# simeonjunker/retr

Measured on AMD Instinct MI355X. Metric: RefCOCO images/sec (train fwd+bwd) at 1/2/4/8 GPUs; greedy-decode refs/sec, higher is better.
Workload: dtype bf16; 1 GPU; cfg2: ResNet-50 + 6-enc/6-dec d_model 256, 640x640, batch 16/GPU, fwd+CE+bwd+allreduce+clip+AdamW; global_batch=16, seq_len=128, parallelism=dp1

## Files before the change

include/retr_hip.h:

```cpp
#ifndef RETR_HIP_H
#define RETR_HIP_H
#include <stddef.h>
#ifdef __cplusplus
extern "C" {
#endif

#define RETR_DTYPE_F32 0
#define RETR_DTYPE_BF16 1

const char* retr_last_error(void);
int retr_abi_version(void);
void retr_set_seed_base(const unsigned long long* device_ptr);
void retr_set_deterministic(int on);
int retr_get_deterministic(void);
int retr_seed_bump(unsigned long long* device_ptr, unsigned long long delta, void* stream);
int retr_spin_us(float us, void* stream);

int retr_linear_fwd(int dtype, const void* x, long ldx, const void* w, long ldw,
                    const float* bias, void* y, long ldy, int y_f32, int M, int N, int K, int relu,
                    const float* residual, long ldr, float drop_p, unsigned long long seed,
                    void* stream);
int retr_linear_dgrad(int dtype, const void* dy, long lddy, const void* w, long ldw, void* dx,
                      long lddx, int dx_f32, int M, int N, int K, const void* addend,
                      int addend_f32, long lda, const void* gate, long ldg, int w_trans,
                      void* stream);
int retr_linear_splits(int dtype, int M, int N, int K);
int retr_linear_fwd_splitk(int dtype, const void* x, long ldx, const void* w, long ldw,
                           const float* bias, void* y, long ldy, int y_f32, int M, int N, int K,
                           int relu, const float* residual, long ldr, float drop_p,
                           unsigned long long seed, float* ws, int splits, void* stream);

typedef struct retr_ln_out {
  const float* gamma;
  const float* beta;
  float eps;
  int y_bf16;
  void* y;
  void* y2;
  long ldy;
  const float* pos;
  int period;
  float* mean;
  float* rstd;
} retr_ln_out;
int retr_linear_fwd_splitk_ln(int dtype, const void* x, long ldx, const void* w, long ldw,
                              const float* bias, float* y, long ldy, int M, int N, int K, int relu,
                              const float* residual, long ldr, float drop_p,
                              unsigned long long seed, float* ws, int splits,
                              const retr_ln_out* ln, void* stream);
int retr_linear_dgrad_splitk(int dtype, const void* dy, long lddy, const void* w, long ldw,
                             void* dx, long lddx, int dx_f32, int M, int N, int K,
                             const void* addend, int addend_f32, long lda, const void* gate,
                             long ldg, int w_trans, float* ws, int splits, void* stream);
int retr_linear_dgrad_slabs(int dtype, const void* dy, long lddy, const void* w, long ldw, int M,
                            int N, int K, int w_trans, float* ws, int splits, void* stream);
int retr_linear_wgrad(int dtype, const void* dy, long lddy, const void* x, long ldx, float* dw,
                      long lddw, int M, int N, int K, float* db, int accumulate, void* stream);
int retr_bias_grad(int dtype, const void* dy, long lddy, int M, int N, float* db, void* stream);

enum {
  RETR_TUNE_GROUP_TILE = 0,
  RETR_TUNE_GROUP_STAGES = 1,
  RETR_TUNE_WGRAD_TILE = 2,
  RETR_TUNE_WGRAD_STAGES = 3,
  RETR_TUNE_WGRAD_KC = 4,
  RETR_TUNE_ATTN_MODE = 5,
  RETR_TUNE_BIG_TILE = 6,
  RETR_TUNE_NT_STORE = 7,
  RETR_TUNE_CONV_WGRAD_SPLITS = 8,
  RETR_TUNE_CONV_WGRAD_TILE = 9,
  RETR_TUNE_ATTN_SPLIT = 10,
  RETR_TUNE_LIN_WGRAD = 11,
  RETR_TUNE_ATTN_FSPLIT = 12,
  RETR_TUNE_LIN_SMALL = 13,
  RETR_TUNE_SHORTK = 14,
  RETR_TUNE_ADAMW_NT = 15,
  RETR_TUNE_WGRAD_B32 = 16,
  RETR_TUNE_WGRAD_FUSED = 17,
  RETR_TUNE_SPLITK_FUSED = 18,
  RETR_TUNE_WB_CHUNK = 19,
  RETR_TUNE_CW_CHUNK = 20,
  RETR_TUNE_CONV3X3 = 21,
  RETR_TUNE_C3_TILE = 22,
  RETR_TUNE_PANEL = 23,
  RETR_TUNE_PANEL_GROUPS = 24,
  RETR_TUNE_PANEL_CONV = 25,
  RETR_TUNE_ATTN_KEEPPRE = 26,
  RETR_TUNE_LN_BWD = 27,
  RETR_TUNE_UNPACK_GRID = 28,
  RETR_TUNE_CW_WAVES = 29,
  RETR_TUNE_DEC_ORDER = 30,
  RETR_TUNE_DEC_WAVES = 31,
  RETR_TUNE_ROWLN = 32,
  RETR_TUNE_LIN_K256 = 33,
  RETR_TUNE_COUNT = 40
};
int retr_tune(int knob, int value);

typedef struct {
  const void* x; long ldx;
  const void* w; long ldw;
  const float* bias;
  void* y; long ldy;
  const float* residual; long ldr;
  float drop_p; unsigned long long seed;
  int M, N, K, relu;
} retr_linear_fwd_desc;
int retr_linear_fwd_group(int dtype, int y_f32, int n, const retr_linear_fwd_desc* d,
                          void* stream);

typedef struct {
  const void* dy; long lddy;
  const void* w; long ldw;
  void* dx; long lddx;
  const void* addend; long lda;
  const void* gate; long ldg;
  int M, N, K, pad;
} retr_linear_dgrad_desc;
int retr_linear_dgrad_group(int dtype, int dx_f32, int addend_f32, int w_trans, int n,
                            const retr_linear_dgrad_desc* d, void* stream);

typedef struct {
  const void* dy; long lddy;
  const void* x; long ldx;
  float* dw; long lddw;
  float* db;
  int M, N, K, accumulate;
} retr_linear_wgrad_desc;
size_t retr_linear_wgrad_group_workspace(int n, const retr_linear_wgrad_desc* d);
int retr_linear_wgrad_group(int dtype, int n, const retr_linear_wgrad_desc* d, void* workspace,
                            void* stream);
typedef struct {
  const float* parts;
  long stride;
  int nparts, cols;
  float* dst;
  int accumulate;
} retr_slab_sum_desc;
int retr_linear_wgrad_group2(int dtype, int n, const retr_linear_wgrad_desc* d, void* workspace,
                             int nx, const retr_slab_sum_desc* x, void* stream);
size_t retr_linear_wgrad_batch_table_bytes(int n, int nx);
int retr_linear_wgrad_batch(int n, const retr_linear_wgrad_desc* d, int nx,
                            const retr_slab_sum_desc* x, void* table, size_t table_bytes,
                            void* stream);

int retr_ffn_splits(int M, int C, int F);
int retr_ffn_fwd(const void* n, long ldn, const void* w1, const float* b1, const void* w2,
                 const float* b2, void* h, long ldh, const float* residual, long ldr, float* y,
                 long ldy, int M, int C, int F, float drop_p, unsigned long long seed, float* ws,
                 int splits, void* stream);
int retr_ffn_bwd_data(const void* dbr, long lddbr, const void* w2, const void* h, long ldh,
                      const void* w1, void* dh, long lddh, void* dn, long lddn, int M, int C,
                      int F, float* ws, int splits, void* stream);

int retr_conv_pack(int dtype, const float* w, const float* bn_w, const float* bn_b,
                   const float* bn_rm, const float* bn_rv, const float* conv_bias, int Co, int Ci,
                   int KH, int KW, int Cp, void* w_out, void* wt_out, float* bias_out,
                   float* scale_out, void* stream);
typedef struct {
  const float *w, *bn_w, *bn_b, *bn_rm, *bn_rv, *conv_bias;
  void *w_out, *wt_out;
  float *bias_out, *scale_out;
  int Co, Ci, KH, KW, Cp, pad;
} retr_conv_pack_desc;
int retr_conv_pack_group(int dtype, int n, const retr_conv_pack_desc* d, void* stream);
typedef struct {
  const void *a, *b;
  void* dst;
  const float *bias_a, *bias_b;
  float* bias_dst;
  int rows, ka, kb;
} retr_cat_rows_desc;
int retr_cat_rows_group(int n, const retr_cat_rows_desc* d, void* stream);
int retr_conv2d_fwd(int dtype, const void* x, int Nb, int H, int W, int C, const void* w,
                    const float* bias, const void* residual, void* y, int Co, int KH, int KW,
                    int stride, int pad, int dil, int relu, void* stream);
int retr_conv2d_fwd_out(int dtype, const void* x, int Nb, int H, int W, int C, const void* w,
                        const float* bias, const void* residual, void* y, int Co, int KH, int KW,
                        int stride, int pad, int dil, int OH, int OW, int relu, void* stream);
int retr_conv1x1_fwd_cat(int dtype, const void* x1, int C1, const void* x2, int C2, int Nb,
                         int OH, int OW, int H2, int W2, int stride2, const void* w,
                         const float* bias, void* y, int Co, int relu, void* stream);
int retr_conv2d_dgrad(int dtype, const void* dy, int Nb, int H, int W, int C, const void* wt,
                      void* dx, int Co, int KH, int KW, int stride, int pad, int dil,
                      const void* addend, const void* gate, void* stream);
int retr_conv2d_wgrad(int dtype, const void* dy, const void* x, int Nb, int H, int W, int C,
                      float* ws, int Co, int KH, int KW, int stride, int pad, int dil,
                      void* stream);
int retr_conv2d_wgrad_splits(int dtype, int Nb, int H, int W, int C, int Co, int KH, int KW,
                             int stride, int pad, int dil);
typedef struct {
  const void* dy; const void* x;
  float* ws;
  int Nb, H, W, C, Co, KH, KW, stride, pad, dil;
  int splits, kind;
} retr_conv_wgrad_desc;
size_t retr_conv2d_wgrad_group_table_bytes(int n);
int retr_conv2d_wgrad_group_plan(int dtype, int n, retr_conv_wgrad_desc* d);
int retr_conv2d_wgrad_group(int dtype, int n, const retr_conv_wgrad_desc* d, void* table,
                            size_t table_bytes, void* stream);
typedef struct {
  const float* ws; const float* scale;
  float* grad;
  int Co, Ci, Cp, KH, KW, splits, accumulate, pad;
} retr_conv_unpack_desc;
size_t retr_conv_wgrad_unpack_group_table_bytes(int n);
int retr_conv_wgrad_unpack_group(int n, const retr_conv_unpack_desc* d, void* table,
                                 size_t table_bytes, void* stream);
int retr_conv_wgrad_unpack(const float* ws, const float* scale, float* grad, int Co, int Ci,
                           int Cp, int KH, int KW, int accumulate, int splits, void* stream);
int retr_bottleneck_s1_fwd(int dtype, const void* x, int N, int H, int W, int Cin,
                           const void* w1, const float* b1, const void* w2, const float* b2,
                           const void* w3, const float* b3, int ds, void* y, void* stream);
int retr_stem_pool_fwd(int dtype, const void* x, int N, int H2, int W2, const void* w,
                       const float* bias, void* y, int Co, void* stream);
int retr_nchw_to_nhwc(int dtype, const float* x, void* y, int N, int C, int H, int W, int Cp,
                      void* stream);
int retr_nchw_to_s2d16(const float* x, void* y, int N, int C, int H, int W, void* stream);
int retr_stem_s2d_weights(const void* wp, void* w2, int Co, int Cp, void* stream);
typedef struct {
  long long src_off;
  long long tmp_off;
  int H, W;
  int x0, y0, rw, rh;
  int bx, by, bw, bh;
  int D, ox, oy;
  int mx, my;
  int coef_off, ksize;
  int win_off;
  int ops;
  float f[3];
  int pad_[2];
} retr_pipe_item;
int retr_pipe_run(const unsigned char* src, const retr_pipe_item* items, int n, const int* coef,
                  const int* win, unsigned char* tmp, int max_d, unsigned char* u8, float* out,
                  unsigned char* mask, int S, const float* mean, const float* std_,
                  void* stream);
int retr_maxpool3x3s2(int dtype, const void* x, void* y, int N, int H, int W, int C, int OH,
                      int OW, void* stream);
int retr_mask_nearest(const unsigned char* m, unsigned char* out, int N, int H, int W, int h,
                      int w, void* stream);

int retr_layernorm_fwd(int dtype, const float* x, long ldx, const float* gamma,
                       const float* beta, float eps, int M, int C, void* y, long ldy, void* y2,
                       const float* pos, int period, float* mean, float* rstd, void* stream);
int retr_layernorm_bwd(int dtype, const void* dy, const void* dy2, long lddy, const float* x,
                       long ldx, const float* gamma, const float* mean, const float* rstd, int M,
                       int C, float* dx, long lddx, const float* addend, float* dgamma,
                       float* dbeta, float* workspace, void* stream);
size_t retr_layernorm_bwd_workspace(int M, int C);
int retr_layernorm_bwd2(int dtype, const void* dy, const void* dy2, long lddy, const float* x,
                        long ldx, const float* gamma, const float* mean, const float* rstd, int M,
                        int C, float* dx, long lddx, const float* addend, float* dgamma,
                        float* dbeta, float* workspace, void* dxd, long lddxd, float drop_p,
                        unsigned long long seed, int* nparts, void* stream);
int retr_layernorm_bwd_slabs(const float* ws, int splits, const float* x, long ldx,
                             const float* gamma, const float* mean, const float* rstd, int M,
                             int C, float* dx, long lddx, const float* addend, float* dgamma,
                             float* dbeta, float* workspace, void* dxd, long lddxd, float drop_p,
                             unsigned long long seed, int* nparts, void* stream);

int retr_embed_ln_fwd(const long long* tokens, int B, int T, int C, const float* word,
                      const float* posw, const float* gamma, const float* beta, float eps,
                      float drop_p, unsigned long long seed, float* y, float* mean, float* rstd,
                      void* stream);
int retr_embed_ln_bwd(const long long* tokens, int B, int T, int C, const float* word,
                      const float* posw, const float* gamma, const float* mean, const float* rstd,
                      const float* dy, float drop_p, unsigned long long seed, float* dword,
                      float* dposw, float* dgamma, float* dbeta, int padding_idx,
                      void* workspace, void* stream);
size_t retr_embed_ln_bwd_workspace(int B, int T, int C);

int retr_attention_fwd(int dtype, const void* q, long ldq, const void* k, long ldk,
                       const void* v, long ldv, void* o, long ldo, int B, int H, int Lq, int Lk,
                       int hd, const unsigned char* kpm, int causal, float drop_p,
                       unsigned long long seed, float* lse, float* probs, void* stream);
int retr_attention_bwd(int dtype, const void* q, long ldq, const void* k, long ldk,
                       const void* v, long ldv, const void* o, long ldo, const void* dout,
                       long lddo, const float* lse, void* dq, long lddq, void* dk, long lddk,
                       void* dv, long lddv, int B, int H, int Lq, int Lk, int hd,
                       const unsigned char* kpm, int causal, float drop_p,
                       unsigned long long seed, float* workspace, void* stream);
size_t retr_attention_bwd_workspace(int B, int H, int Lq);
size_t retr_attention_dropout_mask_bytes(int B, int H, int Lq, int Lk);
int retr_attention_fwd_dm(int dtype, const void* q, long ldq, const void* k, long ldk,
                          const void* v, long ldv, void* o, long ldo, int B, int H, int Lq,
                          int Lk, int hd, const unsigned char* kpm, int causal, float drop_p,
                          unsigned long long seed, float* lse, float* probs, void* dmask,
                          void* stream);
int retr_attention_bwd_dm(int dtype, const void* q, long ldq, const void* k, long ldk,
                          const void* v, long ldv, const void* o, long ldo, const void* dout,
                          long lddo, const float* lse, void* dq, long lddq, void* dk, long lddk,
                          void* dv, long lddv, int B, int H, int Lq, int Lk, int hd,
                          const unsigned char* kpm, int causal, float drop_p,
                          unsigned long long seed, float* workspace, const void* dmask,
                          void* stream);
int retr_attention_decode(int dtype, const void* q, long ldq, const void* k, long ldk,
                          const void* v, long ldv, void* o, long ldo, int B, int H, int Lk,
                          int Lmax, int hd, const unsigned char* kpm, int kv_group,
                          const int* anc, void* stream);

int retr_ce_fwd(int dtype, const void* logits, long ld, int M, int V, const long long* targets,
                float* lse, float* loss_rows, float* loss, void* stream);
int retr_ce_bwd(int dtype, const void* logits, long ld, int M, int V, const long long* targets,
                const float* lse, const float* dloss, float inv_count, void* dlogits, long lddl,
                void* stream);
int retr_ce_fwd_bwd(int dtype, const void* logits, long ld, int M, int V,
                    const long long* targets, float* lse, float* loss_rows, float* loss,
                    float inv_count, void* dlogits, long lddl, void* stream);
int retr_ce_bwd_rescale(int dtype, const void* logits, long ld, int M, int V,
                        const long long* targets, const float* lse, const float* dloss,
                        float inv_count, void* dlogits, long lddl, void* stream);
int retr_ce_count(int M, const long long* targets, long long ignore_index, float* denom,
                  void* stream);
int retr_ce_fwd_opt(int dtype, const void* logits, long ld, int M, int V,
                    const long long* targets, long long ignore_index, float label_smoothing,
                    float* lse, float* loss_rows, float* loss, const float* denom,
                    void* stream);
int retr_ce_bwd_opt(int dtype, const void* logits, long ld, int M, int V,
                    const long long* targets, long long ignore_index, float label_smoothing,
                    const float* lse, const float* dloss, long dloss_stride, const float* denom,
                    void* dlogits, long lddl, void* stream);
int retr_ce_fwd_bwd_opt(int dtype, const void* logits, long ld, int M, int V,
                        const long long* targets, long long ignore_index, float label_smoothing,
                        float* lse, float* loss_rows, float* loss, const float* denom,
                        void* dlogits, long lddl, void* stream);
int retr_ce_bwd_rescale_opt(int dtype, const void* logits, long ld, int M, int V,
                            const long long* targets, long long ignore_index,
                            float label_smoothing, const float* lse, const float* dloss,
                            const float* denom, void* dlogits, long lddl, void* stream);
int retr_argmax_rows(int dtype, const void* x, long ld, int M, int V, long long* out,
                     void* stream);
size_t retr_argmax_workspace(int M);
int retr_argmax_rows_ws(int dtype, const void* x, long ld, int M, int V, long long* out,
                        void* workspace, void* stream);

int retr_topk_rows(int dtype, const void* x, long ld, int M, int V, int K, int* idx,
                   float* logprob, void* stream);
int retr_beam_select(const int* cand_tok, const float* cand_lp, int B, int K, int i, int T,
                     long long eos, float* scores, unsigned char* finished, long long* hist,
                     int* anc, long long* tok, unsigned char* item_done, int* done,
                     void* stream);
int retr_greedy_update(const long long* pred, int B, int T, int i, long long eos,
                       long long* caption, unsigned char* finished, int* done, long long* tok,
                       void* stream);
int retr_greedy_select(int dtype, const void* logits, long ld, int B, int V, void* workspace,
                       int T, int i, long long eos, long long* pred, long long* caption,
                       unsigned char* finished, int* done, long long* tok, void* stream);
int retr_greedy_select2(int dtype, const void* logits, long ld, int B, int V, void* workspace,
                        int T, int i, long long eos, long long* pred, long long* caption,
                        unsigned char* finished, int* done, long long* tok, int write_all,
                        void* stream);

int retr_add_pos_fwd(int dtype, const float* x, long ldx, int M, int C, const float* pos,
                     int period, void* y, void* y2, long ldy, void* stream);
int retr_sum2(int dtype, const void* a, const void* b, long n, float* out, void* stream);
int retr_dropout_apply(int dtype_out, const float* x, long ldx, void* y, long ldy, int M, int N,
                       float drop_p, unsigned long long seed, void* stream);
int retr_transpose_cast(int dtype, const float* x, void* y, int R, int C, int R_pad,
                        void* stream);
int retr_cast(int dtype, const float* x, void* y, long n, void* stream);
int retr_pos_grad(int dtype, const void* d, long ld, int M, int C, int period, float* dpos,
                  void* stream);
int retr_pos_grad_set(int dtype, const void* d, long ld, int M, int C, int period, float* dpos,
                      void* stream);
typedef struct retr_pos_item {
  const void* d;
  long ld;
  int M;
  int pad;
} retr_pos_item;
int retr_pos_grad_multi(int dtype, int n, const retr_pos_item* items, int C, int period,
                        float* dpos, int accumulate, void* stream);

int retr_adamw_sumsq(const float* grad, long n, float* partials, int nparts, float* step,
                     void* stream);
int retr_adamw_update(float* param, float* grad, float* exp_avg, float* exp_avg_sq, long n,
                      const float* hyper, double beta1, double beta2, float eps,
                      const float* step, float step_offset, const float* partials, int nparts,
                      float max_norm, void* param_bf16, void* stream);
int retr_adamw_update2(float* param, float* grad, float* exp_avg, float* exp_avg_sq, long n,
                       const float* hyper, double beta1, double beta2, float eps,
                       const float* step, float step_offset, const float* partials, int nparts,
                       float max_norm, void* param_bf16, int zero_grad, void* stream);

int retr_dec_gemm(const void* a_plain, const void* a_pos, int R, int C, const void* w,
                  const float* bias, int N, void* d0, long rs0, int pos0, void* d1, long rs1,
                  int pos1, void* d2, long rs2, int pos2, int segw, int relu, void* stream);
int retr_dec_rows(const float* xin, const float* slabs, int nslab, const float* b2, int R, int C,
                  float* xout, const float* gamma, const float* beta, float eps, const float* pos,
                  void* n, void* npos, void* stream);
int retr_dec_embed_rows(const long long* tok, int R, int C, const float* word, const float* qpos,
                        const float* ge, const float* be, float epse, float* x, const float* g1,
                        const float* b1, float eps1, void* n, void* npos, void* stream);
int retr_dec_attn_row(const void* q, const void* k, const void* v, int R, int C, int H, int Lk,
                      int Lmax, int kv_group, const int* anc, const unsigned char* kpm,
                      const float* x, const void* wo, const float* bo, float* xo,
// ... 82 lines not shown
```

retr_amd/csrc/conv.hip:

```cpp
#include <algorithm>
#include <cstring>
#include <vector>

#include "gemm2.hpp"
#include "panel.hpp"
#include "epilogues.hpp"
#include "../../include/retr_hip.h"

using namespace retr;

namespace retr {
bool conv3x3_direct_ok(int H, int W, int CI, int CO);
int conv3x3_fwd_direct(const bf16* x, const bf16* w, const float* bias, bf16* y, int relu, int Nb,
                       int H, int W, int CI, int CO, hipStream_t st);
int conv3x3_dgrad_direct(const bf16* dy, const bf16* wt, bf16* dx, const bf16* addend,
                         const bf16* gate, int Nb, int H, int W, int CI_out, int CO_in,
                         hipStream_t st);
}

namespace {

struct Geom {
  int Nb, H, W, C, Co, KH, KW, s, p, d, OH, OW;
};
// ... 245 lines not shown
    int hw = g.OH * g.OW;
    const int n = m / hw;
    int rem = m - n * hw;
    k.oh = rem / g.OW;
    k.ow = rem - k.oh * g.OW;
    k.base = (((long)n * g.H + k.oh * g.s) * g.W + k.ow * g.s) * g.C;
    return k;
  }
  RETR_DEVICE void advance(KCur& k, int d) const {
    k.m += d;
    if (d != Elem<T>::BK) {
      k = kcur(k.m);
      return;
    }
    const long rowC = (long)g.s * g.W * g.C;
    k.ow += adv_r;
    k.oh += adv_q;
    k.base += (long)adv_q * rowC + (long)adv_r * g.s * g.C;
    if (k.ow >= g.OW) {
      k.ow -= g.OW;
      k.oh += 1;
      k.base += rowC - (long)g.OW * g.s * g.C;
    }
    while (k.oh >= g.OH) {
      k.oh -= g.OH;
      k.base += ((long)g.H - (long)g.OH * g.s) * g.W * g.C;
    }
  }
  RETR_DEVICE const void* addr(const Ctx& c, const KCur& k) const {
    if (!c.ok || k.m >= M) return nullptr;
    int ih = k.oh * g.s + c.khd, iw = k.ow * g.s + c.kwd;
    if ((unsigned)ih >= (unsigned)g.H || (unsigned)iw >= (unsigned)g.W) return nullptr;
    return x + k.base + c.off;
  }
};

template <typename T>
struct ConvWgradB32 {
  static constexpr bool kContig = false;
  const T* x;
  Geom g;
  int rows, M;
  int adv_q, adv_r;
  int d_step, d_row, d_img;
  struct Ctx { int khd, kwd, off; bool ok; };
  struct KCur { int m, oh, ow, base; };
  RETR_DEVICE Ctx row_ctx(int r) const {
    Ctx c;
    c.ok = r < rows;
    const int rr = c.ok ? r : 0;
    const int khw = rr / g.C;
    const int ci = rr - khw * g.C;
    const int kh = khw / g.KW, kw = khw - kh * g.KW;
    c.khd = kh * g.d - g.p;
    c.kwd = kw * g.d - g.p;
    c.off = (c.khd * g.W + c.kwd) * g.C + ci;
    return c;
  }
  RETR_DEVICE KCur kcur(int m) const {
    KCur k;
    k.m = m;
    const int hw = g.OH * g.OW;
    const int n = m / hw;
    const int rem = m - n * hw;
    k.oh = rem / g.OW;
    k.ow = rem - k.oh * g.OW;
    k.base = ((n * g.H + k.oh * g.s) * g.W + k.ow * g.s) * g.C;
    return k;
  }
  RETR_DEVICE void advance(KCur& k, int d) const {
    if (d != Elem<T>::BK) {
      k = kcur(k.m + d);
      return;
    }
    k.m += d;
    k.ow += adv_r;
    k.oh += adv_q;
    k.base += d_step;
    if (k.ow >= g.OW) {
      k.ow -= g.OW;
      k.oh += 1;
      k.base += d_row;
    }
    if (k.oh >= g.OH) {
      k.oh -= g.OH;
      k.base += d_img;
    }
  }
  RETR_DEVICE bool ok(const Ctx& c, const KCur& k) const {
    const int ih = k.oh * g.s + c.khd, iw = k.ow * g.s + c.kwd;
    return c.ok & (k.m < M) & ((unsigned)ih < (unsigned)g.H) & ((unsigned)iw < (unsigned)g.W);
  }
  RETR_DEVICE const void* addr(const Ctx& c, const KCur& k) const {
    return ok(c, k) ? (const void*)(x + (unsigned)(k.base + c.off)) : nullptr;
  }
  RETR_DEVICE const void* addr_or(const Ctx& c, const KCur& k, const void* fb) const {
    return ok(c, k) ? (const void*)(x + (unsigned)(k.base + c.off)) : fb;
  }
};

struct Phase {
  int a, b;
  int ih0, iw0;
  int Hp, Wp;
  int nkh, nkw;
};

template <typename T>
struct ConvDgradPhaseA {
  static constexpr bool kContig = true;
  const T* gr;
  Geom g;
  Phase ph;
  int M, K;
  struct Ctx { const T* img; int i, j; bool ok; };
  struct KCur { int k, c, ti, tj; };
  RETR_DEVICE Ctx row_ctx(int r) const {
    Ctx c;
    c.ok = r < M;
    const int rr = c.ok ? r : 0;
    const int hw = ph.Hp * ph.Wp;
    const int n = rr / hw, rem = rr - n * hw;
    c.i = rem / ph.Wp;
    c.j = rem - c.i * ph.Wp;
    c.img = gr + (long)n * g.OH * g.OW * g.Co;
    return c;
  }
  RETR_DEVICE KCur kcur(int k) const {
    KCur t;
    t.k = k;
    const int tap = k / g.Co;
    t.c = k - tap * g.Co;
    t.ti = tap / ph.nkw;
    t.tj = tap - t.ti * ph.nkw;
    return t;
  }
  RETR_DEVICE void advance(KCur& t, int d) const {
    t.k += d;
    t.c += d;
    while (t.c >= g.Co) {
      t.c -= g.Co;
      if (++t.tj == ph.nkw) {
        t.tj = 0;
        ++t.ti;
      }
    }
  }
  RETR_DEVICE const void* addr(const Ctx& c, const KCur& t) const {
    if (!c.ok || t.k >= K) return nullptr;
    const int oh = c.i + ((ph.ih0 + g.p - ph.a) >> 1) - t.ti;
    const int ow = c.j + ((ph.iw0 + g.p - ph.b) >> 1) - t.tj;
    if ((unsigned)oh >= (unsigned)g.OH || (unsigned)ow >= (unsigned)g.OW) return nullptr;
    return c.img + ((long)oh * g.OW + ow) * g.Co + t.c;
  }
};

template <typename T>
struct ConvDgradPhaseAU {
  static constexpr bool kContig = true;
  static constexpr bool kUniformK = true;
  const T* gr;
  Geom g;
  Phase ph;
  int M, K;
  struct Ctx { const T* base; unsigned mask; };
  struct KCur { int c0, t, ti, tj, off; };
  RETR_DEVICE Ctx row_ctx_c(int r, int coff) const {
    Ctx c;
    const bool ok = r < M;
    const int rr = ok ? r : 0;
    const int hw = ph.Hp * ph.Wp;
    const int n = rr / hw, rem = rr - n * hw;
    const int i = rem / ph.Wp, j = rem - i * ph.Wp;
    const int oh0 = i + ((ph.ih0 + g.p - ph.a) >> 1), ow0 = j + ((ph.iw0 + g.p - ph.b) >> 1);
    c.base = gr + (((long)n * g.OH + oh0) * g.OW + ow0) * g.Co + coff;
    unsigned m = 0;
    if (ok) {
      for (int ti = 0; ti < ph.nkh; ++ti)
        for (int tj = 0; tj < ph.nkw; ++tj)
          if ((unsigned)(oh0 - ti) < (unsigned)g.OH && (unsigned)(ow0 - tj) < (unsigned)g.OW)
            m |= 1u << (ti * ph.nkw + tj);
    }
    c.mask = m;
    return c;
  }
  RETR_DEVICE Ctx row_ctx(int r) const { return row_ctx_c(r, 0); }
  RETR_DEVICE void set_off(KCur& t) const { t.off = t.c0 - (t.ti * g.OW + t.tj) * g.Co; }
  RETR_DEVICE KCur kcur(int k) const {
    KCur t;
    t.t = k / g.Co;
    t.c0 = k - t.t * g.Co;
    t.ti = t.t / ph.nkw;
    t.tj = t.t - t.ti * ph.nkw;
    set_off(t);
    return t;
  }
  RETR_DEVICE void advance(KCur& t, int d) const {
    t.c0 += d;
    if (t.c0 >= g.Co) {
      t.c0 -= g.Co;
      ++t.t;
      if (++t.tj == ph.nkw) {
        t.tj = 0;
        ++t.ti;
      }
    }
    set_off(t);
  }
  RETR_DEVICE const void* addr(const Ctx& c, const KCur& t) const {
    if (!((c.mask >> t.t) & 1u)) return nullptr;
    return c.base + t.off;
  }
  RETR_DEVICE const void* addr_or(const Ctx& c, const KCur& t, const void* fb) const {
    return ((c.mask >> t.t) & 1u) ? (const void*)(c.base + t.off) : fb;
  }
};

template <typename T>
struct DgradPhaseWU {
  static constexpr bool kContig = true;
  static constexpr bool kUniformK = true;
  const T* wt;
  Geom g;
  Phase ph;
  int rows, K;
  struct Ctx { const T* row; int klim; };
  struct KCur { int k, c0, ti, tj, off; };
  RETR_DEVICE Ctx row_ctx_c(int r, int coff) const {
    return Ctx{wt + (long)(r < rows ? r : 0) * g.KH * g.KW * g.Co + coff, r < rows ? K : 0};
  }
  RETR_DEVICE Ctx row_ctx(int r) const { return row_ctx_c(r, 0); }
  RETR_DEVICE void set_off(KCur& t) const {
    t.off = ((ph.a + 2 * t.ti) * g.KW + ph.b + 2 * t.tj) * g.Co + t.c0;
  }
  RETR_DEVICE KCur kcur(int k) const {
    KCur t;
    t.k = k;
    const int tap = k / g.Co;
    t.c0 = k - tap * g.Co;
    t.ti = tap / ph.nkw;
    t.tj = tap - t.ti * ph.nkw;
    set_off(t);
    return t;
  }
  RETR_DEVICE void advance(KCur& t, int d) const {
    t.k += d;
    t.c0 += d;
    if (t.c0 >= g.Co) {
      t.c0 -= g.Co;
      if (++t.tj == ph.nkw) {
        t.tj = 0;
        ++t.ti;
      }
    }
    set_off(t);
  }
  RETR_DEVICE const void* addr(const Ctx& c, const KCur& t) const {
    return t.k < c.klim ? (const void*)(c.row + t.off) : nullptr;
  }
  RETR_DEVICE const void* addr_or(const Ctx& c, const KCur& t, const void* fb) const {
    return t.k < c.klim ? (const void*)(c.row + t.off) : fb;
  }
};

template <typename T>
struct DgradPhaseW {
  static constexpr bool kContig = true;
  const T* wt;
  Geom g;
  Phase ph;
  int rows, K;
  struct Ctx { const T* row; bool ok; };
  struct KCur { int k, c, ti, tj; };
  RETR_DEVICE Ctx row_ctx(int r) const {
    return Ctx{wt + (long)(r < rows ? r : 0) * g.KH * g.KW * g.Co, r < rows};
  }
  RETR_DEVICE KCur kcur(int k) const {
    KCur t;
    t.k = k;
    const int tap = k / g.Co;
    t.c = k - tap * g.Co;
    t.ti = tap / ph.nkw;
    t.tj = tap - t.ti * ph.nkw;
    return t;
  }
  RETR_DEVICE void advance(KCur& t, int d) const {
    t.k += d;
    t.c += d;
    while (t.c >= g.Co) {
      t.c -= g.Co;
      if (++t.tj == ph.nkw) {
        t.tj = 0;
        ++t.ti;
      }
    }
  }
  RETR_DEVICE const void* addr(const Ctx& c, const KCur& t) const {
    if (!c.ok || t.k >= K) return nullptr;
    const int kh = ph.a + 2 * t.ti, kw = ph.b + 2 * t.tj;
    return c.row + ((long)kh * g.KW + kw) * g.Co + t.c;
  }
};

template <class EP>
struct EpiPhaseRows {
  EP ep;
  int Hp, Wp, H, W, ih0, iw0;
  static constexpr bool kRowSum = false;
  float* rowsum = nullptr;
  RETR_DEVICE int map(int m) const {
    const int hw = Hp * Wp;
    const int n = m / hw, rem = m - n * hw;
    const int i = rem / Wp, j = rem - i * Wp;
    return (n * H + ih0 + 2 * i) * W + iw0 + 2 * j;
  }
  RETR_DEVICE void apply(int m, int n, float v) const { ep.apply(map(m), n, v); }
  RETR_DEVICE void apply8(int m, int n, float (&v)[8]) const { ep.apply8(map(m), n, v); }
  using Pre = typename EP::Pre;
  RETR_DEVICE void fetch8(int m, int n, Pre& p) const { ep.fetch8(map(m), n, p); }
  RETR_DEVICE void apply8p(int m, int n, float (&v)[8], const Pre& p) const {
    ep.apply8p(map(m), n, v, p);
  }
  RETR_DEVICE void empty_split(int, int) const {}
  RETR_DEVICE bool lane_contiguous() const { return false; }
};

inline bool prefer_tile64(int M, int N, int K, bool dense1x1, bool res_small_k) {
  if (retr_tune_get(RETR_TUNE_BIG_TILE) != 0) return false;
  if (res_small_k) return true;
  if (M <= 8192 && (N <= 512 || K <= 512)) return true;
  return dense1x1 && N >= 1024 && K <= 512 && M <= 32768;
}

template <int FAM, typename T, class LA, class LB, class EP>
int launch_auto(const LA& la, const LB& lb, const EP& ep, int M, int N, int K, int splits,
                hipStream_t st, const char* what, bool dense1x1 = false,
                bool res_small_k = false) {
  if constexpr (sizeof(T) == 2) {
    return launch_big<FAM>(la, lb, ep, M, N, K, splits, st, what,
                           prefer_tile64(M, N, K, dense1x1, res_small_k));
  } else {
    if (N >= 128 && M >= 4096) return launch_gemm<FAM, T, 128, 128>(la, lb, ep, M, N, K, splits, st, what);
    return launch_gemm<FAM, T, 64, 64>(la, lb, ep, M, N, K, splits, st, what);
  }
}

struct WgradPlan {
  int tile;
  int splits;
};

template <typename T>
WgradPlan wgrad_plan(int R, int Ncols, int Mp, bool dense1x1) {
  constexpr int BK = Elem<T>::BK;
  WgradPlan p{64, 1};
  if (R >= 128 && Ncols >= 128) p.tile = sizeof(T) == 2 ? 128 : 129;
  const int tt = retr_tune_get(RETR_TUNE_CONV_WGRAD_TILE);
  if (sizeof(T) == 2 && R >= 64 && Ncols >= 64 &&
      (tt == 1 || (tt == 0 && dense1x1 && (R <= 128 || Ncols <= 128 || Mp <= 8192))))
    p.tile = 65;
  if (p.tile == 65 && tt == 3) p.tile = 66;
  const int bm = (p.tile == 64 || p.tile == 65 || p.tile == 66) ? 64 : 128;
  const int bn = bm;
  const long tiles = (long)cdiv(R, bm) * cdiv(Ncols, bn);
  const int ksteps = cdiv(Mp, BK);
  const int tune = retr_tune_get(RETR_TUNE_CONV_WGRAD_SPLITS);
  long smax = ksteps / 8;
  if (smax > 128) smax = 128;
  if (smax < 1) smax = 1;
  long s;
  if (tune >= 2) {
    s = tune < smax ? tune : smax;
  } else if (tune == 1 || (p.tile != 128 && p.tile != 65 && p.tile != 66)) {
    s = (512 + tiles - 1) / tiles;
    if (s > smax) s = smax;
  } else {
    const long slots = p.tile == 66 ? 2048 : p.tile == 65 ? 1024 : 512;
    const double slab_cost = p.tile == 128 ? 0.016 : 0.004;
    s = 1;
    double best = 1e30;
    for (long c = 1; c <= smax; ++c) {
      const long kc = cdiv(ksteps, (int)c);
      const long rounds = (tiles * cdiv(ksteps, (int)kc) + slots - 1) / slots;
      const double cost = (double)rounds * (kc + 2) + slab_cost * (double)tiles * c;
      if (cost < best) { best = cost; s = c; }
    }
  }
  if (s < 1) s = 1;
  const int kchunk = cdiv(ksteps, (int)s) * BK;
  p.splits = cdiv(Mp, kchunk);
  return p;
}

template <int FAM, typename T, class LA, class LB>
int launch_wgrad(const LA& la, const LB& lb, float* ws, long ldws, int R, int Ncols, int Mp,
                 hipStream_t st, const char* what, bool dense1x1) {
  const WgradPlan p = wgrad_plan<T>(R, Ncols, Mp, dense1x1);
  const int s = p.splits;
  EpiAccF32 ep{ws, ldws, 0, 0, 1, nullptr};
  ep.split_stride = s > 1 ? (long)R * ldws : 0;
  ep.set_vec();
  if constexpr (sizeof(T) == 2) {
    if (p.tile == 128 && !dense1x1)
      return launch_gemm2<FAM, 128, 128, 4, 2, 2>(la, lb, ep, R, Ncols, Mp, s, st, what);
    if (p.tile == 128) return launch_gemm2<FAM, 128, 128, 2, 2, 2>(la, lb, ep, R, Ncols, Mp, s, st, what);
    if (p.tile == 65) return launch_gemm2<FAM, 64, 64, 2, 2, 2>(la, lb, ep, R, Ncols, Mp, s, st, what);
    if (p.tile == 66) return launch_gemm2<FAM, 64, 64, 2, 2, 1>(la, lb, ep, R, Ncols, Mp, s, st, what);
  } else {
    if (p.tile == 129) return launch_gemm<FAM, T, 128, 128>(la, lb, ep, R, Ncols, Mp, s, st, what);
  }
  return launch_gemm<FAM, T, 64, 64>(la, lb, ep, R, Ncols, Mp, s, st, what);
}

template <typename T>
int conv_fwd_t(const void* x, Geom g, const void* w, const float* bias, const void* res, void* y,
               int relu, hipStream_t st) {
  int M = g.Nb * g.OH * g.OW, N = g.Co, K = g.KH * g.KW * g.C;
  DenseK<T> lb{(const T*)w, (long)K, N, K};
  EpiFwd<T, T> ep{(T*)y, (long)N, bias, (const T*)res, (long)N, relu ? 2 : 0, DropoutParams{0, 0, 1.f}, 0};
  ep.set_vec();
  if (g.KH == 1 && g.KW == 1 && g.s == 1 && g.p == 0) {
    DenseK<T> la{(const T*)x, (long)g.C, M, K};
    if constexpr (sizeof(T) == 2) {
      if (K <= 256 && K % 64 == 0 && N >= 1024 && retr_tune_get(RETR_TUNE_PANEL) == 1 &&
          retr_tune_get(RETR_TUNE_PANEL_CONV) == 1)
        return launch_panel<kFamConvFwd>(la, lb, ep, M, N, K, st, "conv_fwd_1x1");
    }
    return launch_auto<kFamConvFwd, T>(la, lb, ep, M, N, K, 1, st, "conv_fwd_1x1", true,
                                       res != nullptr && K <= 64);
  }
  if constexpr (sizeof(T) == 2) {
    if (g.KH == 3 && g.KW == 3 && g.s == 1 && g.p == 1 && g.d == 1 && !res && relu &&
        conv3x3_direct_ok(g.H, g.W, g.C, g.Co))
      return conv3x3_fwd_direct((const bf16*)x, (const bf16*)w, bias, (bf16*)y, relu, g.Nb, g.H,
                                g.W, g.C, g.Co, st);
  }
  if (sizeof(T) == 2 && g.C % 64 == 0 && g.KH * g.KW > 1 && g.KH * g.KW <= 32) {
    ConvFwdAU<T> la{(const T*)x, g, M, K};
    return launch_auto<kFamConvFwd, T>(la, lb, ep, M, N, K, 1, st, "conv_fwd");
  }
  ConvFwdA<T> la{(const T*)x, g, M, K};
  return launch_auto<kFamConvFwd, T>(la, lb, ep, M, N, K, 1, st, "conv_fwd");
}

__global__ void dgrad_phase_fill_kernel(bf16* dx, const bf16* addend, const bf16* gate, int H,
                                        int W, int C, long chunks, int zmask) {
  const long i = blockIdx.x * (long)blockDim.x + threadIdx.x;
  if (i >= chunks) return;
  const int cpp = C / 8;
  const long p = i / cpp;
  const int c = (int)(i - p * cpp) * 8;
  const int iw = (int)(p % W), ih = (int)((p / W) % H);
  if (!((zmask >> ((ih & 1) * 2 + (iw & 1))) & 1)) return;
  const long off = p * C + c;
  bf16x8 v;
  if (addend) {
    v = *(const bf16x8*)(addend + off);
  } else {
#pragma unroll
    for (int e = 0; e < 8; ++e) v[e] = (bf16)0.f;
  }
  if (gate) {
    const bf16x8 gg = *(const bf16x8*)(gate + off);
#pragma unroll
    for (int e = 0; e < 8; ++e)
      if (!((float)gg[e] > 0.f)) v[e] = (bf16)0.f;
  }
  *(bf16x8*)(dx + off) = v;
}

template <typename T>
int conv_dgrad_t(const void* dy, Geom g, const void* wt, void* dx, const void* addend,
                 const void* gate, hipStream_t st) {
  int M = g.Nb * g.H * g.W, N = g.C, K = g.KH * g.KW * g.Co;
  DenseK<T> lb{(const T*)wt, (long)K, N, K};
  EpiDgrad<T, T, T> ep{(T*)dx, (long)N, (const T*)addend, (long)N, (const T*)gate, (long)N};
  ep.set_vec();
  if (g.KH == 1 && g.KW == 1 && g.s == 1 && g.p == 0) {
    DenseK<T> la{(const T*)dy, (long)g.Co, M, K};
    if constexpr (sizeof(T) == 2) {
      if (K <= 256 && K % 64 == 0 && N >= 1024 && retr_tune_get(RETR_TUNE_PANEL) == 1 &&
          retr_tune_get(RETR_TUNE_PANEL_CONV) == 1)
        return launch_panel<kFamConvDgrad>(la, lb, ep, M, N, K, st, "conv_dgrad_1x1");
    }
    return launch_auto<kFamConvDgrad, T>(la, lb, ep, M, N, K, 1, st, "conv_dgrad_1x1", true);
  }
  if (g.s == 2 && g.d == 1) {
    int zmask = 0;
    for (int a = 0; a < 2; ++a)
      for (int bb = 0; bb < 2; ++bb) {
        const int nkh = g.KH > a ? (g.KH - a + 1) / 2 : 0;
        const int nkw = g.KW > bb ? (g.KW - bb + 1) / 2 : 0;
        if (nkh * nkw == 0) {
          const int ih0 = ((a - g.p) % 2 + 2) % 2, iw0 = ((bb - g.p) % 2 + 2) % 2;
          zmask |= 1 << (ih0 * 2 + iw0);
        }
      }
    const bool inplace = addend != nullptr && addend == dx;
    if (zmask && (inplace || (sizeof(T) == 2 && N % 8 == 0))) {
      if (!inplace) {
        const long chunks = (long)M * (N / 8);
        hipLaunchKernelGGL(dgrad_phase_fill_kernel, dim3((unsigned)cdiv(chunks, 256)), dim3(256),
                           0, st, (bf16*)dx, (const bf16*)addend, (const bf16*)gate, g.H, g.W, N,
                           chunks, zmask);
        if (int e = retr_check_launch("conv_dgrad_phase_fill")) return e;
      }
    } else {
      zmask = 0;
    }
    for (int a = 0; a < 2; ++a)
      for (int bb = 0; bb < 2; ++bb) {
        Phase ph;
        ph.a = a;
        ph.b = bb;
        ph.ih0 = ((a - g.p) % 2 + 2) % 2;
        ph.iw0 = ((bb - g.p) % 2 + 2) % 2;
        ph.Hp = g.H > ph.ih0 ? (g.H - ph.ih0 + 1) / 2 : 0;
        ph.Wp = g.W > ph.iw0 ? (g.W - ph.iw0 + 1) / 2 : 0;
        ph.nkh = g.KH > a ? (g.KH - a + 1) / 2 : 0;
        ph.nkw = g.KW > bb ? (g.KW - bb + 1) / 2 : 0;
        const int Mp = g.Nb * ph.Hp * ph.Wp, Kp = ph.nkh * ph.nkw * g.Co;
        if (Mp == 0) continue;
        if (Kp == 0 && (zmask >> (ph.ih0 * 2 + ph.iw0) & 1)) continue;
        EpiPhaseRows<EpiDgrad<T, T, T>> pe{ep, ph.Hp, ph.Wp, g.H, g.W, ph.ih0, ph.iw0};
        if (sizeof(T) == 2 && g.Co % 64 == 0 && ph.nkh * ph.nkw <= 32) {
          ConvDgradPhaseAU<T> pa{(const T*)dy, g, ph, Mp, Kp};
          DgradPhaseWU<T> pb{(const T*)wt, g, ph, N, Kp};
          if constexpr (sizeof(T) == 2) {
            if (N <= 128 && Mp >= 65536 && retr_tune_get(RETR_TUNE_BIG_TILE) == 0 &&
                retr_tune_get(RETR_TUNE_SHORTK) != 1) {
              if (int e = launch_gemm2<kFamConvDgrad, 64, 128, 2, 2, 1>(pa, pb, pe, Mp, N, Kp, 1,
                                                                          st, "conv_dgrad_s2"))
                return e;
              continue;
            }
          }
          if (int e = launch_auto<kFamConvDgrad, T>(pa, pb, pe, Mp, N, Kp, 1, st, "conv_dgrad_s2"))
            return e;
          continue;
        }
        ConvDgradPhaseA<T> pa{(const T*)dy, g, ph, Mp, Kp};
        DgradPhaseW<T> pb{(const T*)wt, g, ph, N, Kp};
        if (int e = launch_auto<kFamConvDgrad, T>(pa, pb, pe, Mp, N, Kp, 1, st, "conv_dgrad_s2"))
          return e;
      }
    return 0;
  }
  if constexpr (sizeof(T) == 2) {
    if (g.KH == 3 && g.KW == 3 && g.s == 1 && g.p == 1 && g.d == 1 &&
        conv3x3_direct_ok(g.H, g.W, g.Co, g.C))
      return conv3x3_dgrad_direct((const bf16*)dy, (const bf16*)wt, (bf16*)dx,
                                  (const bf16*)addend, (const bf16*)gate, g.Nb, g.H, g.W, g.Co,
                                  g.C, st);
  }
  if (sizeof(T) == 2 && g.s == 1 && g.Co % 64 == 0 && g.KH * g.KW <= 32) {
    ConvDgradAU<T> la{(const T*)dy, g, M, K};
    return launch_auto<kFamConvDgrad, T>(la, lb, ep, M, N, K, 1, st, "conv_dgrad");
  }
  ConvDgradA<T> la{(const T*)dy, g, M, K};
  return launch_auto<kFamConvDgrad, T>(la, lb, ep, M, N, K, 1, st, "conv_dgrad");
}

template <typename T>
int conv_wgrad_t(const void* dy, const void* x, Geom g, float* ws, hipStream_t st) {
  int Mp = g.Nb * g.OH * g.OW;
  int R = g.Co, Ncols = g.KH * g.KW * g.C;
  DenseT<T> la{(const T*)dy, (long)g.Co, R, Mp};
  if (g.KH == 1 && g.KW == 1 && g.s == 1 && g.p == 0) {
    DenseT<T> lb{(const T*)x, (long)g.C, Ncols, Mp};
    return launch_wgrad<kFamConvWgrad, T>(la, lb, ws, (long)Ncols, R, Ncols, Mp, st, "conv_wgrad_1x1",
                                          true);
  }
  constexpr int BK = Elem<T>::BK;
  if constexpr (sizeof(T) == 2) {
    if ((long)g.Nb * g.H * g.W * g.C < (1L << 31) && g.OH * g.OW >= BK &&
        retr_tune_get(RETR_TUNE_WGRAD_B32) != 1) {
      const int q = BK / g.OW, r = BK % g.OW;
      ConvWgradB32<T> lb{(const T*)x, g, Ncols, Mp, q, r,
                         (q * g.s * g.W + r * g.s) * g.C,
                         g.s * g.W * g.C - g.OW * g.s * g.C,
                         (g.H - g.OH * g.s) * g.W * g.C};
      return launch_wgrad<kFamConvWgrad, T>(la, lb, ws, (long)Ncols, R, Ncols, Mp, st,
                                            "conv_wgrad", false);
    }
  }
  ConvWgradB<T> lb{(const T*)x, g, Ncols, Mp, BK / g.OW, BK % g.OW};
  return launch_wgrad<kFamConvWgrad, T>(la, lb, ws, (long)Ncols, R, Ncols, Mp, st, "conv_wgrad", false);
}

template <typename T>
__global__ void conv_pack_kernel(const float* w, const float* bnw, const float* bnb,
                                 const float* bnrm, const float* bnrv, const float* conv_bias,
                                 int Co, int Ci, int KH, int KW, int Cp, T* wout, T* wtout,
                                 float* bias_out, float* scale_out) {
  long total = (long)Co * KH * KW * Cp;
  for (long i = blockIdx.x * (long)blockDim.x + threadIdx.x; i < total;
       i += (long)gridDim.x * blockDim.x) {
    int ci = i % Cp;
    long t = i / Cp;
    int kw = t % KW;
    t /= KW;
    int kh = t % KH;
    int co = (int)(t / KH);
    float scale = 1.f;
    if (bnw) scale = bnw[co] * (1.0f / sqrtf(bnrv[co] + 1e-5f));
    float v = ci < Ci ? w[(((long)co * Ci + ci) * KH + kh) * KW + kw] * scale : 0.f;
    wout[i] = from_f<T>(v);
    if (wtout) wtout[(((long)ci * KH + kh) * KW + kw) * Co + co] = from_f<T>(v);
    if (ci == 0 && kh == 0 && kw == 0) {
      float b;
      if (bnw) b = bnb[co] - bnrm[co] * scale;
      else b = conv_bias ? conv_bias[co] : 0.f;
      if (bias_out) bias_out[co] = b;
      if (scale_out) scale_out[co] = scale;
    }
  }
}

__global__ void wgrad_unpack4_kernel(const float* ws, const float* scale, float* grad, int Co,
                                     int Ci, int Cp, int KHW, int accumulate, int splits) {
  const int c4 = Ci / 4;
  const long total = (long)Co * KHW * c4;
  const long slab = (long)Co * KHW * Cp;
  for (long i = blockIdx.x * (long)blockDim.x + threadIdx.x; i < total;
       i += (long)gridDim.x * blockDim.x) {
    const int ci = (int)(i % c4) * 4;
    const long t = i / c4;
    const int tap = (int)(t % KHW), co = (int)(t / KHW);
    const float* src = ws + ((long)co * KHW + tap) * Cp + ci;
    f32x4 v = *(const f32x4*)src;
    int s = 1;
    for (; s + 7 < splits; s += 8) {
      f32x4 u[8];
#pragma unroll
      for (int k = 0; k < 8; ++k) u[k] = *(const f32x4*)(src + (s + k) * slab);
#pragma unroll
      for (int k = 0; k < 8; ++k) v += u[k];
    }
    for (; s < splits; ++s) v += *(const f32x4*)(src + s * slab);
    const float sc = scale ? scale[co] : 1.f;
    float* dst = grad + ((long)co * Ci + ci) * KHW + tap;
#pragma unroll
    for (int e = 0; e < 4; ++e) {
      const float x = v[e] * sc;
      dst[(long)e * KHW] = accumulate ? dst[(long)e * KHW] + x : x;
    }
  }
}

template <int NW>
__global__ void __launch_bounds__(NW * 64)
wgrad_unpack4w_kernel(const float* ws, const float* scale, float* grad, int Co, int Ci, int Cp,
                      int KHW, int accumulate, int splits) {
  __shared__ f32x4 red[NW][64];
  const int lane = threadIdx.x & 63, w = threadIdx.x >> 6;
  const int c4 = Ci / 4;
  const long total = (long)Co * KHW * c4;
  const long slab = (long)Co * KHW * Cp;
  const long i = (long)blockIdx.x * 64 + lane;
  int ci = 0, tap = 0, co = 0;
  f32x4 v = {0.f, 0.f, 0.f, 0.f};
  if (i < total) {
    ci = (int)(i % c4) * 4;
    const long t = i / c4;
    tap = (int)(t % KHW);
    co = (int)(t / KHW);
    const float* src = ws + ((long)co * KHW + tap) * Cp + ci;
    int s = w;
    for (; s + 7 * NW < splits; s += 8 * NW) {
      f32x4 u[8];
#pragma unroll
      for (int k = 0; k < 8; ++k) u[k] = *(const f32x4*)(src + (long)(s + k * NW) * slab);
#pragma unroll
      for (int k = 0; k < 8; ++k) v += u[k];
    }
    for (; s < splits; s += NW) v += *(const f32x4*)(src + (long)s * slab);
  }
  if constexpr (NW > 1) {
    red[w][lane] = v;
    __syncthreads();
    if (w != 0) return;
#pragma unroll
    for (int k = 1; k < NW; ++k) v += red[k][lane];
  }
  if (i >= total) return;
  const float sc = scale ? scale[co] : 1.f;
  float* dst = grad + ((long)co * Ci + ci) * KHW + tap;
#pragma unroll
  for (int e = 0; e < 4; ++e) {
    const float x = v[e] * sc;
    dst[(long)e * KHW] = accumulate ? dst[(long)e * KHW] + x : x;
  }
}

__global__ void wgrad_unpack_kernel(const float* ws, const float* scale, float* grad, int Co,
                                    int Ci, int Cp, int KH, int KW, int accumulate, int splits) {
  const long total = (long)Co * Ci * KH * KW;
  const long slab = (long)Co * KH * KW * Cp;
  for (long i = blockIdx.x * (long)blockDim.x + threadIdx.x; i < total;
       i += (long)gridDim.x * blockDim.x) {
    int kw = i % KW;
    long t = i / KW;
    int kh = t % KH;
    t /= KH;
    int ci = t % Ci;
    int co = (int)(t / Ci);
    const long src = ((long)co * KH * KW + kh * KW + kw) * Cp + ci;
    float v = ws[src];
    int s = 1;
    for (; s + 7 < splits; s += 8) {
      float t[8];
#pragma unroll
      for (int u = 0; u < 8; ++u) t[u] = ws[src + (s + u) * slab];
#pragma unroll
      for (int u = 0; u < 8; ++u) v += t[u];
    }
    for (; s < splits; ++s) v += ws[src + s * slab];
    if (scale) v *= scale[co];
    grad[i] = accumulate ? grad[i] + v : v;
  }
}

constexpr int kPackGroup = 16;
constexpr int kPackPerThread = 4;

struct PackGroup {
  retr_conv_pack_desc d[kPackGroup];
  int blk0[kPackGroup + 1];
  int n;
};

template <typename T>
__global__ void __launch_bounds__(256) conv_pack_group_kernel(PackGroup g) {
  const int bid = blockIdx.x;
  int p = 0;
#pragma unroll
  for (int i = 1; i < kPackGroup; ++i)
    if (i < g.n && bid >= g.blk0[i]) p = i;
  const retr_conv_pack_desc& d = g.d[p];
  const int Co = d.Co, Ci = d.Ci, KH = d.KH, KW = d.KW, Cp = d.Cp;
  const long total = (long)Co * KH * KW * Cp;
  const long base = ((long)(bid - g.blk0[p]) * 256 + threadIdx.x) * kPackPerThread;
  const float* bnw = d.bn_w;
#pragma unroll
  for (int u = 0; u < kPackPerThread; ++u) {
    const long i = base + u;
    if (i >= total) break;
    const int ci = (int)(i % Cp);
    long t = i / Cp;
    const int kw = (int)(t % KW);
    t /= KW;
    const int kh = (int)(t % KH);
    const int co = (int)(t / KH);
    float scale = 1.f;
    if (bnw) scale = bnw[co] * (1.0f / sqrtf(d.bn_rv[co] + 1e-5f));
    const float v = ci < Ci ? d.w[(((long)co * Ci + ci) * KH + kh) * KW + kw] * scale : 0.f;
    ((T*)d.w_out)[i] = from_f<T>(v);
    if (d.wt_out) ((T*)d.wt_out)[(((long)ci * KH + kh) * KW + kw) * Co + co] = from_f<T>(v);
    if (ci == 0 && kh == 0 && kw == 0) {
      float b;
      if (bnw) b = d.bn_b[co] - d.bn_rm[co] * scale;
      else b = d.conv_bias ? d.conv_bias[co] : 0.f;
      if (d.bias_out) d.bias_out[co] = b;
      if (d.scale_out) d.scale_out[co] = scale;
    }
  }
}

template <typename T, int KHW>
__global__ void __launch_bounds__(256) conv_pack_tiled_group_kernel(PackGroup g) {
  extern __shared__ __attribute__((aligned(16))) char smem[];
  T* tile = (T*)smem;
  __shared__ float sc[64];
  const int bid = blockIdx.x;
  int p = 0;
#pragma unroll
  for (int i = 1; i < kPackGroup; ++i)
    if (i < g.n && bid >= g.blk0[i]) p = i;
  const retr_conv_pack_desc& d = g.d[p];
  const int Co = d.Co, Cp = d.Cp;
  const int t = bid - g.blk0[p], tn = Cp / 64;
  const int co0 = (t / tn) * 64, ci0 = (t % tn) * 64;
  const int tid = threadIdx.x;
  if (tid < 64) {
    const int co = co0 + tid;
    float scale = 1.f;
    if (d.bn_w) scale = d.bn_w[co] * (1.0f / sqrtf(d.bn_rv[co] + 1e-5f));
    sc[tid] = scale;
    if (ci0 == 0) {
      float b;
      if (d.bn_w) b = d.bn_b[co] - d.bn_rm[co] * scale;
      else b = d.conv_bias ? d.conv_bias[co] : 0.f;
      if (d.bias_out) d.bias_out[co] = b;
      if (d.scale_out) d.scale_out[co] = scale;
    }
  }
  __syncthreads();
  constexpr int ROW = 64 * KHW;
  constexpr int LDR = ROW + 2;
  constexpr int TOT = 64 * ROW;
  constexpr int R4 = ROW / 4;
  static_assert(ROW % 4 == 0, "pack row");
#pragma unroll 4
  for (int f = tid; f < 64 * R4; f += 256) {
    const int r = f / R4, j = 4 * (f - r * R4);
    const float4 v = *(const float4*)(d.w + ((long)(co0 + r) * Cp + ci0) * KHW + j);
    const float s = sc[r];
    tile[r * LDR + j] = from_f<T>(v.x * s);
    tile[r * LDR + j + 1] = from_f<T>(v.y * s);
    tile[r * LDR + j + 2] = from_f<T>(v.z * s);
    tile[r * LDR + j + 3] = from_f<T>(v.w * s);
  }
  __syncthreads();
  constexpr int VEC = 16 / sizeof(T), NV = 64 / VEC;
  typedef __attribute__((ext_vector_type(4))) unsigned int u4;
  T* wout = (T*)d.w_out;
#pragma unroll 4
  for (int e = tid; e < 64 * KHW * NV; e += 256) {
    const int cc = e % NV, q = e / NV;
    const int tap = q % KHW, r = q / KHW;
    T v[VEC];
#pragma unroll
    for (int k = 0; k < VEC; ++k) v[k] = tile[r * LDR + (cc * VEC + k) * KHW + tap];
    *(u4*)(wout + ((long)(co0 + r) * KHW + tap) * Cp + ci0 + cc * VEC) = *(const u4*)v;
  }
  if (!d.wt_out) return;
  T* wt = (T*)d.wt_out;
#pragma unroll 4
  for (int e = tid; e < 64 * KHW * NV; e += 256) {
    const int rc = e % NV, q = e / NV;
    const int tap = q % KHW, ci = q / KHW;
    T v[VEC];
#pragma unroll
    for (int k = 0; k < VEC; ++k) v[k] = tile[(rc * VEC + k) * LDR + ci * KHW + tap];
    *(u4*)(wt + ((long)(ci0 + ci) * KHW + tap) * Co + co0 + rc * VEC) = *(const u4*)v;
  }
}

Geom make_geom(int Nb, int H, int W, int C, int Co, int KH, int KW, int s, int p, int d) {
  Geom g{Nb, H, W, C, Co, KH, KW, s, p, d, 0, 0};
  g.OH = (H + 2 * p - d * (KH - 1) - 1) / s + 1;
  g.OW = (W + 2 * p - d * (KW - 1) - 1) / s + 1;
  return g;
}


struct CWProb {
  const bf16* dy;
// ... 633 lines not shown
```

Baseline: 1717 images/s.

## Group stride-2 conv dgrad phase GEMMs into one launch and use fast division

The four sub-pixel phase GEMMs of a stride-2 conv backward-data, previously launched one after another, are now batched into a single grouped kernel. Phases are sorted by K so the longest ones are scheduled first, and the tile shape is chosen from N and Co. The row-mapping epilogue swaps integer division for multiply-shift fast division and caches the mapped row between the fetch and apply steps. This removes launch overhead and tail underutilization of small per-phase grids, at the cost of a new tuning knob and possibly less suited tile shapes for some layers.

```diff
diff --git a/include/retr_hip.h b/include/retr_hip.h
--- a/include/retr_hip.h
+++ b/include/retr_hip.h
@@ -93,6 +93,7 @@
   RETR_TUNE_DEC_WAVES = 31,
   RETR_TUNE_ROWLN = 32,
   RETR_TUNE_LIN_K256 = 33,
+  RETR_TUNE_DGRAD_S2 = 34,
   RETR_TUNE_COUNT = 40
 };
 int retr_tune(int knob, int value);
diff --git a/retr_amd/csrc/conv.hip b/retr_amd/csrc/conv.hip
--- a/retr_amd/csrc/conv.hip
+++ b/retr_amd/csrc/conv.hip
@@ -571,24 +571,49 @@
   }
 };
 
+struct FastDiv {
+  unsigned mul = 0, sh = 0;
+  FastDiv() = default;
+  explicit FastDiv(int d) {
+    if (d <= 1) return;
+    int l = 1;
+    while ((1L << l) < d) ++l;
+    mul = (unsigned)(((1UL << (31 + l)) + (unsigned long)d - 1) / (unsigned long)d);
+    sh = (unsigned)(l - 1);
+  }
+  RETR_DEVICE int div(int x) const {
+    return mul ? (int)(__umulhi((unsigned)x, mul) >> sh) : x;
+  }
+};
+
 template <class EP>
 struct EpiPhaseRows {
   EP ep;
   int Hp, Wp, H, W, ih0, iw0;
+  FastDiv dhw, dw;
   static constexpr bool kRowSum = false;
   float* rowsum = nullptr;
+  EpiPhaseRows() = default;
+  EpiPhaseRows(const EP& e, int hp, int wp, int h, int w, int i0, int j0)
+      : ep(e), Hp(hp), Wp(wp), H(h), W(w), ih0(i0), iw0(j0), dhw(hp * wp), dw(wp) {}
   RETR_DEVICE int map(int m) const {
     const int hw = Hp * Wp;
-    const int n = m / hw, rem = m - n * hw;
-    const int i = rem / Wp, j = rem - i * Wp;
+    const int n = dhw.div(m), rem = m - n * hw;
+    const int i = dw.div(rem), j = rem - i * Wp;
     return (n * H + ih0 + 2 * i) * W + iw0 + 2 * j;
   }
   RETR_DEVICE void apply(int m, int n, float v) const { ep.apply(map(m), n, v); }
   RETR_DEVICE void apply8(int m, int n, float (&v)[8]) const { ep.apply8(map(m), n, v); }
-  using Pre = typename EP::Pre;
-  RETR_DEVICE void fetch8(int m, int n, Pre& p) const { ep.fetch8(map(m), n, p); }
-  RETR_DEVICE void apply8p(int m, int n, float (&v)[8], const Pre& p) const {
-    ep.apply8p(map(m), n, v, p);
+  struct Pre {
+    typename EP::Pre p;
+    int row;
+  };
+  RETR_DEVICE void fetch8(int m, int n, Pre& p) const {
+    p.row = map(m);
+    ep.fetch8(p.row, n, p.p);
+  }
+  RETR_DEVICE void apply8p(int, int n, float (&v)[8], const Pre& p) const {
+    ep.apply8p(p.row, n, v, p.p);
   }
   RETR_DEVICE void empty_split(int, int) const {}
   RETR_DEVICE bool lane_contiguous() const { return false; }
@@ -738,6 +763,65 @@
   *(bf16x8*)(dx + off) = v;
 }
 
+struct DgradS2Phase {
+  ConvDgradPhaseAU<bf16> a;
+  DgradPhaseWU<bf16> b;
+  EpiPhaseRows<EpiDgrad<bf16, bf16, bf16>> e;
+  int M, K;
+};
+
+template <int FAM, int BM, int BN, int WM, int WN, int S, int EPB, class LA, class LB, class EP>
+__global__ void __launch_bounds__(WM * WN * 64)
+dgrad_s2_gemm2_group_kernel(GGroup<LA, LB, EP, 4> g) {
+  const int bid = xcd_remap(blockIdx.x, gridDim.x);
+  const int tn = g.p[0].tiles_n, per = g.n * tn;
+  const int tm = bid / per, r = bid - tm * per;
+  const int p = r / tn;
+  const GProb<LA, LB, EP>& d = g.p[p];
+  const int tile = tm * tn + (r - p * tn);
+  if (tile >= d.tiles) return;
+  gemm2_tile<FAM, BM, BN, WM, WN, S, EPB>(d.la, d.lb, d.ep, d.M, d.N, d.K, d.kchunk, d.tiles_n,
+                                          tile, 0);
+}
+
+template <int BM, int BN, int WM, int WN, int S>
+int dgrad_s2_group_launch(const DgradS2Phase* ph, int n, int N, hipStream_t st) {
+  using LA = ConvDgradPhaseAU<bf16>;
+  using LB = DgradPhaseWU<bf16>;
+  using EP = EpiPhaseRows<EpiDgrad<bf16, bf16, bf16>>;
+  Group2<kFamConvDgrad, BM, BN, WM, WN, S, 0, LA, LB, EP, 4> grp;
+  static_assert(sizeof(grp.g) < 4096, "dgrad_s2 group: kernel-argument space");
+  int tm_max = 0;
+  for (int i = 0; i < n; ++i) {
+    if (grp.add(ph[i].a, ph[i].b, ph[i].e, ph[i].M, N, ph[i].K, 1)) return 1;
+    tm_max = std::max(tm_max, cdiv(ph[i].M, BM));
+  }
+  constexpr size_t lds = gemm2_lds_bytes<BM, BN, S, 0>();
+  auto kern = dgrad_s2_gemm2_group_kernel<kFamConvDgrad, BM, BN, WM, WN, S, 0, LA, LB, EP>;
+  if constexpr (lds > 65536) {
+    static bool attr_set = false;
+    if (!attr_set) {
+      (void)hipFuncSetAttribute((const void*)kern, hipFuncAttributeMaxDynamicSharedMemorySize,
+                                (int)lds);
+      attr_set = true;
+    }
+  }
+  hipLaunchKernelGGL(kern, dim3(tm_max * n * cdiv(N, BN)), dim3(WM * WN * 64), lds, st, grp.g);
+  return retr_check_launch("conv_dgrad_s2_group");
+}
+
+int dgrad_s2_group(DgradS2Phase* ph, int n, int N, int Co, int knob, hipStream_t st) {
+  std::stable_sort(ph, ph + n,
+                   [](const DgradS2Phase& x, const DgradS2Phase& y) { return x.K > y.K; });
+  int tile = knob >= 2 && knob <= 5 ? knob : (N >= 512 && Co >= 512 ? 5 : 3);
+  switch (tile) {
+    case 2: return dgrad_s2_group_launch<64, 64, 2, 2, 2>(ph, n, N, st);
+    case 3: return dgrad_s2_group_launch<64, 64, 2, 2, 1>(ph, n, N, st);
+    case 4: return dgrad_s2_group_launch<64, 128, 2, 2, 1>(ph, n, N, st);
+    default: return dgrad_s2_group_launch<128, 128, 4, 2, 2>(ph, n, N, st);
+  }
+}
+
 template <typename T>
 int conv_dgrad_t(const void* dy, Geom g, const void* wt, void* dx, const void* addend,
                  const void* gate, hipStream_t st) {
@@ -755,11 +839,12 @@
     return launch_auto<kFamConvDgrad, T>(la, lb, ep, M, N, K, 1, st, "conv_dgrad_1x1", true);
   }
   if (g.s == 2 && g.d == 1) {
-    int zmask = 0;
+    int zmask = 0, ntap = 0;
     for (int a = 0; a < 2; ++a)
       for (int bb = 0; bb < 2; ++bb) {
         const int nkh = g.KH > a ? (g.KH - a + 1) / 2 : 0;
         const int nkw = g.KW > bb ? (g.KW - bb + 1) / 2 : 0;
+        ntap += nkh * nkw > 0;
         if (nkh * nkw == 0) {
           const int ih0 = ((a - g.p) % 2 + 2) % 2, iw0 = ((bb - g.p) % 2 + 2) % 2;
           zmask |= 1 << (ih0 * 2 + iw0);
@@ -777,6 +862,12 @@
     } else {
       zmask = 0;
     }
+    const int s2knob = retr_tune_get(RETR_TUNE_DGRAD_S2);
+    const bool grouped = sizeof(T) == 2 && s2knob != 1 && ntap > 1 &&
+                         retr_tune_get(RETR_TUNE_BIG_TILE) == 0 &&
+                         retr_tune_get(RETR_TUNE_SHORTK) != 1;
+    DgradS2Phase gph[4];
+    int ngph = 0;
     for (int a = 0; a < 2; ++a)
       for (int bb = 0; bb < 2; ++bb) {
         Phase ph;
@@ -796,6 +887,10 @@
           ConvDgradPhaseAU<T> pa{(const T*)dy, g, ph, Mp, Kp};
           DgradPhaseWU<T> pb{(const T*)wt, g, ph, N, Kp};
           if constexpr (sizeof(T) == 2) {
+            if (grouped && Kp > 0) {
+              gph[ngph++] = DgradS2Phase{pa, pb, pe, Mp, Kp};
+              continue;
+            }
             if (N <= 128 && Mp >= 65536 && retr_tune_get(RETR_TUNE_BIG_TILE) == 0 &&
                 retr_tune_get(RETR_TUNE_SHORTK) != 1) {
               if (int e = launch_gemm2<kFamConvDgrad, 64, 128, 2, 2, 1>(pa, pb, pe, Mp, N, Kp, 1,
@@ -813,6 +908,7 @@
         if (int e = launch_auto<kFamConvDgrad, T>(pa, pb, pe, Mp, N, Kp, 1, st, "conv_dgrad_s2"))
           return e;
       }
+    if (ngph) return dgrad_s2_group(gph, ngph, N, g.Co, s2knob, st);
     return 0;
   }
   if constexpr (sizeof(T) == 2) {
```

Result: no change. 1730 images/s, median of 6 (+0.8%).
